# Aster32/GAN-DANet

Hardware: AMD Instinct MI355X
Metric: train samples/sec (G+D step) on 256x256 tiles (higher is better)
Workload: dtype bf16; 1 GPU; full G+D train step, 8ch 256x256 -> 1024x1024 tiles, batch 32/GPU (global 32), perceptual=on, SSIM evaluated, AdamW x2; survey_config=3, per_gpu_batch=32, global_batch=32, tile=256, parallelism=dp1

## Files before the change

### gan-danet_amd/_lib.py

```python
from __future__ import annotations

import ctypes as C
import os

HERE = os.path.dirname(os.path.abspath(__file__))
LIB_PATH = os.path.join(HERE, "lib", "libgandanet_hip.so")

PREC_FP32, PREC_BF16, PREC_X3 = 0, 1, 2
PAM_BWD_K64_ATOMIC, PAM_BWD_K64_PARTS, PAM_BWD_K32_PARTS, PAM_BWD_TWO_KERNEL = 0, 1, 2, 3
ACT_NONE, ACT_RELU, ACT_LEAKY02, ACT_SIGMOID = 0, 1, 2, 3
EVAL_F64, EVAL_SKIP_NAN = 1, 2
GUARD_SQNORM, GUARD_NORM, GUARD_COEF, GUARD_OK, GUARD_APPLIED, GUARD_SKIPPED, GUARD_RECORD = range(7)
GUARD_CHUNK = 65536
FILTER_F32, FILTER_F64 = 0, 1
EDGE_REFLECT, EDGE_INTERIOR = 0, 1
FILTER_MAX_RADIUS, SAVGOL_MAX_WINDOW = 64, 33
ZOOM_MIRROR, ZOOM_NEAREST = 0, 1

c_fp = C.c_void_p


class ConvDesc(C.Structure):
    _fields_ = [
        ("B", C.c_int), ("M", C.c_int), ("Mstore", C.c_int), ("Ck", C.c_int), ("ks", C.c_int),
# ... 41 lines not shown
    "gd_gemm_nt_plan": (_i, [C.POINTER(GemmNTDesc), _sz, C.POINTER(_i), C.POINTER(_sz)]),
    "gd_conv3x3_ws_bytes": (_sz, [_i, _i]),
    "gd_conv3x3_eligible": (_i, [C.POINTER(ConvDesc)]),
    "gd_conv3x3": (_i, [C.POINTER(ConvDesc), _p, _sz, _p]),
    "gd_conv3x3_wgrad": (_i, [_p, _l, _p, _p, _l, _p, _i, _p, _p, _i, _i, _i, _i, _i, _i, _i, _i, _p, _p]),
    "gd_conv3x3_wgrad_ws": (_i, [_p, _l, _p, _p, _l, _p, _i, _p, _p, _i, _i, _i, _i, _i, _i, _i, _i, _p, _p, _p, _sz]),
    "gd_conv3x3_wgrad_plan": (_i, [_i, _i, _i, _i, _i, _i, _sz, C.POINTER(_i), C.POINTER(_sz)]),
    "gd_pack_16_split": (_i, [_p, _l, _i, _i, _i, _p, _p, _i, _p, _l, _i, _l, _i, _i, _p, _l, _i, _l, _i, _i, _p]),
    "gd_pack_16_split_masked": (_i, [_p, _l, _i, _i, _i, _p, _p, _i, _p, _l, _i, _l, _i, _i, _p, _l, _i, _l, _i, _i, _p, _l, _p]),
    "gd_split3_weights": (_i, [_p, _l, _l, _l, _p, _p]),
    "gd_bn_stats_ws_floats": (_sz, [_i, _i, _l]),
    "gd_bn_stats": (_i, [_p, _l, _i, _i, _l, _f, _f, _p, _p, _p, _p, _p, _p]),
    "gd_bn_fold": (_i, [_p, _p, _p, _p, _i, _p, _p, _p]),
    "gd_bn_fold_eval": (_i, [_p, _p, _p, _p, _f, _i, _p, _p, _p, _p]),
    "gd_affine_act": (_i, [_p, _l, _p, _p, _i, _i, _l, _i, _p, _l, _p]),
    "gd_bn_act_bwd": (_i, [_p, _l, _p, _l, _p, _p, _p, _p, _p, _i, _i, _l, _i, _i, _p, _p, _p, _l, _i, _p, _p]),
    "gd_bn_stats_local": (_i, [_p, _l, _i, _i, _l, _p, _p, _p]),
    "gd_bn_stats_merge": (_i, [_p, _i, _i, _f, _f, _p, _p, _p, _p, _p]),
    "gd_bn_act_bwd_dx": (_i, [_p, _l, _p, _l, _p, _p, _p, _p, _p, _p, _f, _i, _i, _l, _i, _p, _l, _i, _p]),
    "gd_bicubic_fwd": (_i, [_p, _i, _i, _i, _p, _i, _i, _f, _f, _p]),
    "gd_bicubic_bwd": (_i, [_p, _i, _i, _i, _p, _i, _i, _f, _f, _p]),
    "gd_bilinear_fwd": (_i, [_p, _i, _i, _i, _p, _i, _i, _i, _p, _p]),
    "gd_bilinear_bwd": (_i, [_p, _i, _i, _i, _p, _i, _i, _p]),
    "gd_maxpool2_fwd": (_i, [_p, _i, _i, _i, _p, _p]),
    "gd_maxpool2_bwd": (_i, [_p, _p, _i, _i, _i, _p, _p]),
    "gd_act_fwd": (_i, [_p, _p, _l, _i, _p]),
    "gd_act_bwd": (_i, [_p, _p, _p, _l, _i, _p]),
    "gd_axpby": (_i, [_p, _f, _p, _f, _l, _p]),
    "gd_scale_dev": (_i, [_p, _p, _p, _l, _i, _p]),
    "gd_copy_rows": (_i, [_p, _l, _l, _p, _l, _l, _i, _i, _i, _p]),
    "gd_channel_sum": (_i, [_p, _l, _i, _i, _l, _p, _i, _p, _p]),
    "gd_copy_slab": (_i, [_p, _l, _p, _l, _i, _l, _i, _p]),
    "gd_softmax_rows": (_i, [_p, _p, _l, _i, _f, _p]),
    "gd_softmax_rows_bwd": (_i, [_p, _p, _p, _l, _i, _f, _p]),
# ... 131 lines not shown
```

### gan-danet_amd/csrc/norm.hip

```cpp
#include "common.h"
#include "../../include/gandanet.h"

namespace {

constexpr int CHUNK = 16384;

static inline int chunks_per_image(long HW) { return (int)((HW + CHUNK - 1) / CHUNK); }

__global__ __launch_bounds__(256) void bn_partial_kernel(const float* __restrict__ x, long x_bs, int C, long HW,
                                                        int cpi, float* __restrict__ ws) {
    __shared__ float red[8];
    const int c = blockIdx.x;
    const int part = blockIdx.y;
    const int b = part / cpi, j = part - b * cpi;
    const long i0 = (long)j * CHUNK;
    const long i1 = min(HW, i0 + (long)CHUNK);
    const float* p = x + (long)b * x_bs + (long)c * HW;
    const float shift = p[i0];
    float s1 = 0.f, s2 = 0.f;
    for (long i = i0 + threadIdx.x; i < i1; i += 256) {
        const float v = p[i] - shift;
        s1 += v;
        s2 = fmaf(v, v, s2);
    }
    s1 = gd_block_sum(s1, red);
    s2 = gd_block_sum(s2, red);
    if (threadIdx.x == 0) {
        const float n = (float)(i1 - i0);
        float* o = ws + ((long)c * gridDim.y + part) * 3;
        o[0] = n;
        o[1] = shift + s1 / n;
        o[2] = fmaxf(s2 - s1 * s1 / n, 0.f);
    }
}

__global__ __launch_bounds__(256) void bn_finalize_kernel(const float* __restrict__ ws, int parts, long c_stride,
                                                         long p_stride, float eps, float momentum,
                                                         float* __restrict__ mean, float* __restrict__ invstd,
                                                         float* running_mean, float* running_var,
                                                         float* __restrict__ stats_out) {
    __shared__ double redd[4];
    const int c = blockIdx.x;
    const float* w0 = ws + (long)c * c_stride * 3;
    const long ps = p_stride * 3;
    double n = 0, sm = 0;
    for (int i = threadIdx.x; i < parts; i += 256) {
        const float* w = w0 + i * ps;
        n += w[0];
        sm += (double)w[0] * w[1];
    }
    auto bsum = [&](double v) {
        v = gd_wave_sum_d(v);
        __syncthreads();
// ... 7 lines not shown
    double m2 = 0;
    for (int i = threadIdx.x; i < parts; i += 256) {
        const float* w = w0 + i * ps;
        const double dm = (double)w[1] - mu;
        m2 += (double)w[2] + (double)w[0] * dm * dm;
    }
    m2 = bsum(m2);
    if (threadIdx.x == 0 && stats_out) {
        stats_out[c * 3 + 0] = (float)n;
        stats_out[c * 3 + 1] = (float)mu;
        stats_out[c * 3 + 2] = (float)m2;
    } else if (threadIdx.x == 0) {
        const double var = m2 / n;
        mean[c] = (float)mu;
        invstd[c] = (float)(1.0 / sqrt(var + (double)eps));
        if (running_mean) {
            const double unb = n > 1 ? m2 / (n - 1) : var;
            running_mean[c] = (float)((1.0 - momentum) * running_mean[c] + momentum * mu);
            running_var[c] = (float)((1.0 - momentum) * running_var[c] + momentum * unb);
        }
    }
}

__global__ __launch_bounds__(256) void chan_sum_partial_kernel(const float* __restrict__ x, long x_bs, long HW, int cpi,
                                                              float* __restrict__ ws) {
    __shared__ float red[8];
    const int c = blockIdx.x;
    const int part = blockIdx.y;
    const int b = part / cpi, j = part - b * cpi;
    const long i0 = (long)j * CHUNK, i1 = min(HW, i0 + (long)CHUNK);
    const float* p = x + (long)b * x_bs + (long)c * HW;
    float s = 0.f;
    for (long i = i0 + threadIdx.x; i < i1; i += 256) s += p[i];
    s = gd_block_sum(s, red);
    if (threadIdx.x == 0) ws[(long)c * gridDim.y + part] = s;
// ... 113 lines not shown
    };
    a = bsum(a);
    g = bsum(g);
    if (threadIdx.x == 0) {
        dbeta[c] = (float)a;
        dgamma[c] = (float)g;
    }
}

__global__ __launch_bounds__(256) void bn_bwd_dx_kernel(const float* __restrict__ dy, long dy_bs,
                                                       const float* __restrict__ x, long x_bs,
                                                       const float* __restrict__ scale, const float* __restrict__ shift,
                                                       const float* __restrict__ mean, const float* __restrict__ invstd,
                                                       const float* __restrict__ dgamma, const float* __restrict__ dbeta,
                                                       float inv_n, long HW, int cpi, int act, int train,
                                                       float* __restrict__ dx, long dx_bs, int accumulate) {
    const int c = blockIdx.x;
    const int b = blockIdx.y / cpi, j = blockIdx.y - b * cpi;
    const long i0 = (long)j * CHUNK, i1 = min(HW, i0 + (long)CHUNK);
    const float* px = x + (long)b * x_bs + (long)c * HW;
    const float* pd = dy + (long)b * dy_bs + (long)c * HW;
    float* po = dx + (long)b * dx_bs + (long)c * HW;
    const float sc = scale[c], sh = shift[c], mu = mean[c], is = invstd[c];
    const float k_db = train ? dbeta[c] * inv_n : 0.f;
    const float k_dg = train ? dgamma[c] * inv_n : 0.f;
    for (long i = i0 + threadIdx.x; i < i1; i += 256) {
        const float xv = px[i];
        const float g = act_grad(fmaf(xv, sc, sh), pd[i], act);
        const float xh = (xv - mu) * is;
        float v = sc * (g - k_db - xh * k_dg);
        if (accumulate) v += po[i];
        po[i] = v;
    }
}

}

extern "C" size_t gd_bn_stats_ws_floats(int B, int C, long HW) {
    return (size_t)C * (size_t)B * (size_t)chunks_per_image(HW) * 3;
}

extern "C" int gd_bn_stats(const float* x, long x_bs, int B, int C, long HW, float eps, float momentum, float* mean,
                           float* invstd, float* running_mean, float* running_var, float* ws, void* stream) {
    GD_CHECK_ARG(x && mean && invstd && ws, "gd_bn_stats: null pointer");
    GD_CHECK_ARG(B > 0 && C > 0 && HW > 0, "gd_bn_stats: bad sizes");
    GD_CHECK_ARG((running_mean == nullptr) == (running_var == nullptr), "gd_bn_stats: running stats must come together");
    const int cpi = chunks_per_image(HW);
    GD_CHECK_ARG((long)B * cpi <= 65535, "gd_bn_stats: too many parts");
    hipStream_t s = (hipStream_t)stream;
    hipLaunchKernelGGL(bn_partial_kernel, dim3(C, B * cpi), dim3(256), 0, s, x, x_bs, C, HW, cpi, ws);
    hipLaunchKernelGGL(bn_finalize_kernel, dim3(C), dim3(256), 0, s, ws, B * cpi, (long)B * cpi, 1L, eps, momentum, mean, invstd,
                       running_mean, running_var, (float*)nullptr);
    GD_LAUNCH_CHECK();
    return 0;
}

extern "C" int gd_bn_stats_local(const float* x, long x_bs, int B, int C, long HW, float* stats, float* ws, void* stream) {
    GD_CHECK_ARG(x && stats && ws && B > 0 && C > 0 && HW > 0, "gd_bn_stats_local: bad arguments");
    const int cpi = chunks_per_image(HW);
    GD_CHECK_ARG((long)B * cpi <= 65535, "gd_bn_stats_local: too many parts");
    hipStream_t s = (hipStream_t)stream;
    hipLaunchKernelGGL(bn_partial_kernel, dim3(C, B * cpi), dim3(256), 0, s, x, x_bs, C, HW, cpi, ws);
    hipLaunchKernelGGL(bn_finalize_kernel, dim3(C), dim3(256), 0, s, ws, B * cpi, (long)B * cpi, 1L, 0.f, 0.f, (float*)nullptr,
                       (float*)nullptr, (float*)nullptr, (float*)nullptr, stats);
    GD_LAUNCH_CHECK();
    return 0;
}
extern "C" int gd_bn_stats_merge(const float* stats_all, int world, int C, float eps, float momentum, float* mean,
                                 float* invstd, float* running_mean, float* running_var, void* stream) {
    GD_CHECK_ARG(stats_all && mean && invstd && world > 0 && C > 0, "gd_bn_stats_merge: bad arguments");
    GD_CHECK_ARG((running_mean == nullptr) == (running_var == nullptr), "gd_bn_stats_merge: running stats must come together");
    hipLaunchKernelGGL(bn_finalize_kernel, dim3(C), dim3(256), 0, (hipStream_t)stream, stats_all, world, 1L, (long)C, eps,
                       momentum, mean, invstd, running_mean, running_var, (float*)nullptr);
    GD_LAUNCH_CHECK();
    return 0;
}

extern "C" int gd_channel_sum(const float* x, long x_bs, int B, int C, long HW, float* out, int accumulate, float* ws,
                              void* stream) {
    GD_CHECK_ARG(x && out && ws && B > 0 && C > 0 && HW > 0, "gd_channel_sum: bad arguments");
    const int cpi = chunks_per_image(HW);
    GD_CHECK_ARG((long)B * cpi <= 65535, "gd_channel_sum: too many parts");
    hipStream_t s = (hipStream_t)stream;
    hipLaunchKernelGGL(chan_sum_partial_kernel, dim3(C, B * cpi), dim3(256), 0, s, x, x_bs, HW, cpi, ws);
    hipLaunchKernelGGL(chan_sum_final_kernel, dim3(C), dim3(256), 0, s, ws, B * cpi, out, accumulate);
    GD_LAUNCH_CHECK();
    return 0;
}
// ... 19 lines not shown

extern "C" int gd_affine_act(const float* x, long x_bs, const float* scale, const float* shift, int B, int C, long HW,
                             int act, float* y, long y_bs, void* stream) {
    GD_CHECK_ARG(x && y && B > 0 && C > 0 && HW > 0, "gd_affine_act: bad arguments");
    const int cpi = chunks_per_image(HW);
    GD_CHECK_ARG((long)B * cpi <= 65535, "gd_affine_act: too many parts");
    hipLaunchKernelGGL(affine_act_kernel, dim3(C, B * cpi), dim3(256), 0, (hipStream_t)stream, x, x_bs, scale, shift, HW,
                       cpi, act, y, y_bs);
    GD_LAUNCH_CHECK();
    return 0;
}

extern "C" int gd_bn_act_bwd_dx(const float* dy, long dy_bs, const float* x, long x_bs, const float* scale, const float* shift,
                                const float* mean, const float* invstd, const float* dgamma_sum, const float* dbeta_sum,
                                float inv_n, int B, int C, long HW, int act, float* dx, long dx_bs, int accumulate_dx,
                                void* stream) {
    GD_CHECK_ARG(dy && x && scale && shift && mean && invstd && dgamma_sum && dbeta_sum && dx, "gd_bn_act_bwd_dx: null pointer");
    GD_CHECK_ARG(B > 0 && C > 0 && HW > 0 && inv_n > 0.f, "gd_bn_act_bwd_dx: bad sizes");
    const int cpi = chunks_per_image(HW);
    GD_CHECK_ARG((long)B * cpi <= 65535, "gd_bn_act_bwd_dx: too many parts");
    hipLaunchKernelGGL(bn_bwd_dx_kernel, dim3(C, B * cpi), dim3(256), 0, (hipStream_t)stream, dy, dy_bs, x, x_bs, scale, shift, mean,
                       invstd, dgamma_sum, dbeta_sum, inv_n, HW, cpi, act, 1, dx, dx_bs, accumulate_dx);
    GD_LAUNCH_CHECK();
    return 0;
}

extern "C" int gd_bn_act_bwd(const float* dy, long dy_bs, const float* x, long x_bs, const float* scale,
                             const float* shift, const float* mean, const float* invstd, const float* gamma, int B, int C,
                             long HW, int act, int train, float* dgamma, float* dbeta, float* dx, long dx_bs,
                             int accumulate_dx, float* ws, void* stream) {
    (void)gamma;
    GD_CHECK_ARG(dy && x && scale && shift && mean && invstd && dgamma && dbeta && ws, "gd_bn_act_bwd: null pointer");
    GD_CHECK_ARG(B > 0 && C > 0 && HW > 0, "gd_bn_act_bwd: bad sizes");
    const int cpi = chunks_per_image(HW);
    GD_CHECK_ARG((long)B * cpi <= 65535, "gd_bn_act_bwd: too many parts");
    hipStream_t s = (hipStream_t)stream;
    hipLaunchKernelGGL(bn_bwd_partial_kernel, dim3(C, B * cpi), dim3(256), 0, s, dy, dy_bs, x, x_bs, scale, shift, mean,
                       invstd, HW, cpi, act, ws);
    hipLaunchKernelGGL(bn_bwd_finalize_kernel, dim3(C), dim3(256), 0, s, ws, B * cpi, dgamma, dbeta);
    if (dx) {
        const float inv_n = 1.0f / ((float)B * (float)HW);
        hipLaunchKernelGGL(bn_bwd_dx_kernel, dim3(C, B * cpi), dim3(256), 0, s, dy, dy_bs, x, x_bs, scale, shift, mean,
                           invstd, dgamma, dbeta, inv_n, HW, cpi, act, train, dx, dx_bs, accumulate_dx);
    }
    GD_LAUNCH_CHECK();
    return 0;
}
```

### gan-danet_amd/kern.py

```python
from __future__ import annotations

import ctypes as C
import math
import os
from typing import Optional, Tuple

import torch

from . import _lib as L

Tensor = torch.Tensor


def _stream() -> int:
    return torch.cuda.current_stream().cuda_stream


def _ptr(t: Optional[Tensor]):
    return None if t is None else t.data_ptr()


def _chk(t: Tensor, name: str = "tensor", dtype=torch.float32) -> None:
    if not t.is_cuda:
        raise L.GandanetError(f"{name}: expected a GPU tensor (there is no CPU fallback in the product path)")
# ... 224 lines not shown
    return out


def bn_stats(x: Tensor, eps: float, momentum: float, running_mean: Optional[Tensor],
             running_var: Optional[Tensor]) -> Tuple[Tensor, Tensor]:
    bs = _bview(x, "bn input")
    B, Cn = x.shape[0], x.shape[1]
    HW = x[0, 0].numel()
    mean = torch.empty(Cn, device=x.device, dtype=torch.float32)
    invstd = torch.empty_like(mean)
    L.check(lib().gd_bn_stats(_ptr(x), bs, B, Cn, HW, eps, momentum, _ptr(mean), _ptr(invstd), _ptr(running_mean),
                              _ptr(running_var), _ptr(bn_ws(B, Cn, HW, x.device)), _stream()), "gd_bn_stats")
    return mean, invstd


def bn_stats_local(x: Tensor) -> Tensor:
    bs = _bview(x, "bn input")
    B, Cn = x.shape[0], x.shape[1]
    HW = x[0, 0].numel()
    stats = torch.empty(Cn, 3, device=x.device, dtype=torch.float32)
    L.check(lib().gd_bn_stats_local(_ptr(x), bs, B, Cn, HW, _ptr(stats), _ptr(bn_ws(B, Cn, HW, x.device)), _stream()),
            "gd_bn_stats_local")
    return stats


def bn_stats_merge(stats_all: Tensor, eps: float, momentum: float, running_mean: Optional[Tensor],
                   running_var: Optional[Tensor]) -> Tuple[Tensor, Tensor]:
    _dense(stats_all, "gathered BN records")
    world, Cn, _ = stats_all.shape
    mean = torch.empty(Cn, device=stats_all.device, dtype=torch.float32)
    invstd = torch.empty_like(mean)
    L.check(lib().gd_bn_stats_merge(_ptr(stats_all), world, Cn, eps, momentum, _ptr(mean), _ptr(invstd), _ptr(running_mean),
                                    _ptr(running_var), _stream()), "gd_bn_stats_merge")
    return mean, invstd


def bn_act_bwd_dx(dy: Tensor, x: Tensor, scale: Tensor, shift: Tensor, mean: Tensor, invstd: Tensor, dgamma_sum: Tensor,
                  dbeta_sum: Tensor, inv_n: float, act: int, dx: Optional[Tensor] = None, accumulate_dx: bool = False) -> Tensor:
    dbs, xbs = _bview(dy, "bn dy"), _bview(x, "bn x")
    B, Cn = x.shape[0], x.shape[1]
    HW = x[0, 0].numel()
    if dx is None:
        dx = torch.empty(x.shape, device=x.device, dtype=torch.float32)
        accumulate_dx = False
    L.check(lib().gd_bn_act_bwd_dx(_ptr(dy), dbs, _ptr(x), xbs, _ptr(scale), _ptr(shift), _ptr(mean), _ptr(invstd),
                                   _ptr(dgamma_sum), _ptr(dbeta_sum), float(inv_n), B, Cn, HW, act, _ptr(dx), _bview(dx),
                                   int(accumulate_dx), _stream()), "gd_bn_act_bwd_dx")
    return dx


def bn_fold(gamma: Tensor, beta: Tensor, mean: Tensor, invstd: Tensor) -> Tuple[Tensor, Tensor]:
    scale, shift = torch.empty_like(gamma), torch.empty_like(gamma)
    L.check(lib().gd_bn_fold(_ptr(gamma), _ptr(beta), _ptr(mean), _ptr(invstd), gamma.numel(), _ptr(scale),
                             _ptr(shift), _stream()), "gd_bn_fold")
    return scale, shift


def bn_fold_eval(gamma: Tensor, beta: Tensor, running_mean: Tensor, running_var: Tensor, eps: float):
    scale, shift, invstd = torch.empty_like(gamma), torch.empty_like(gamma), torch.empty_like(gamma)
    L.check(lib().gd_bn_fold_eval(_ptr(gamma), _ptr(beta), _ptr(running_mean), _ptr(running_var), eps,
                                  gamma.numel(), _ptr(scale), _ptr(shift), _ptr(invstd), _stream()), "gd_bn_fold_eval")
    return scale, shift, invstd


def affine_act(x: Tensor, scale: Optional[Tensor], shift: Optional[Tensor], act: int,
               out: Optional[Tensor] = None) -> Tensor:
    bs = _bview(x, "affine input")
    B, Cn = x.shape[0], x.shape[1]
    HW = x[0, 0].numel()
    if out is None:
        out = torch.empty(x.shape, device=x.device, dtype=torch.float32)
    L.check(lib().gd_affine_act(_ptr(x), bs, _ptr(scale), _ptr(shift), B, Cn, HW, act, _ptr(out), _bview(out),
                                _stream()), "gd_affine_act")
    return out


def bn_act_bwd(dy: Tensor, x: Tensor, scale: Tensor, shift: Tensor, mean: Tensor, invstd: Tensor, act: int,
               train: bool, dx: Optional[Tensor] = None, accumulate_dx: bool = False, want_dx: bool = True,
               sums_out: Optional[Tensor] = None):
    dbs, xbs = _bview(dy, "bn dy"), _bview(x, "bn x")
    B, Cn = x.shape[0], x.shape[1]
    HW = x[0, 0].numel()
    if sums_out is not None:
        dgamma, dbeta = _dense(sums_out)[0], sums_out[1]
    else:
        dgamma = torch.empty(Cn, device=x.device, dtype=torch.float32)
        dbeta = torch.empty_like(dgamma)
    if want_dx and dx is None:
        dx = torch.empty(x.shape, device=x.device, dtype=torch.float32)
    L.check(lib().gd_bn_act_bwd(_ptr(dy), dbs, _ptr(x), xbs, _ptr(scale), _ptr(shift), _ptr(mean), _ptr(invstd), None,
                                B, Cn, HW, act, int(train), _ptr(dgamma), _ptr(dbeta), _ptr(dx) if want_dx else None,
                                _bview(dx) if want_dx else 0, int(accumulate_dx), _ptr(bn_ws(B, Cn, HW, x.device)),
                                _stream()), "gd_bn_act_bwd")
    return dgamma, dbeta, dx


def bicubic_fwd(x: Tensor, Ho: int, Wo: int, rsh: float, rsw: float) -> Tensor:
    _dense(x, "bicubic input")
    B, Cn, Hi, Wi = x.shape
    y = torch.empty(B, Cn, Ho, Wo, device=x.device, dtype=torch.float32)
    L.check(lib().gd_bicubic_fwd(_ptr(x), B * Cn, Hi, Wi, _ptr(y), Ho, Wo, rsh, rsw, _stream()), "gd_bicubic_fwd")
    return y


def shift_sum9_fwd(u: Tensor, bias: Optional[Tensor]) -> Tensor:
    _dense(u, "tap planes")
    B, nine, H, W = u.shape
    if nine != 9:
# ... 1120 lines not shown
```

### gan-danet_amd/ops.py

```python
from __future__ import annotations

import os
from typing import List, Optional

import torch
from torch.autograd import Function

from . import _lib as L
from . import kern as K
from .config import config, operand_mode, sixteen_bit

ACT_NONE, ACT_RELU, ACT_LEAKY, ACT_SIGMOID = L.ACT_NONE, L.ACT_RELU, L.ACT_LEAKY02, L.ACT_SIGMOID


def _prec(layer: str = "other") -> int:
    mode = operand_mode(layer)
    return L.PREC_BF16 if mode == "16" else L.PREC_X3 if mode == "x3" else L.PREC_FP32


def _x3(layer: str) -> bool:
    return operand_mode(layer) == "x3"


def _x3_eligible(x, w, stride, pad, act) -> bool:
    return (x.dim() == 4 and tuple(w.shape[2:]) == (3, 3) and stride == 1 and pad == 1 and act in (ACT_NONE, ACT_RELU)
            and w.shape[1] >= 32 and w.shape[1] % 8 == 0 and w.shape[0] % 8 == 0 and (x.shape[2] * x.shape[3]) % 8 == 0
            and x.shape[2] * x.shape[3] * 3 * max(w.shape[0], w.shape[1]) < (1 << 31))


def _pam_f16() -> bool:
    return config.precision in ("fp16", "mixed")


def _c(t: torch.Tensor) -> torch.Tensor:
    return t if t.is_contiguous() else t.contiguous()


DISC_NHWC = os.environ.get("GD_DISC_NHWC", "1") != "0"


def disc1_trunk_eligible(x: torch.Tensor, ws) -> bool:
    return (DISC_NHWC and (sixteen_bit("disc") or _x3("disc")) and (not K.DETERMINISTIC or K.DET_REDUCE == "ordered")
            and x.dim() == 4 and x.shape[1] <= 4
            and ws[0].shape[0] == 64 and all(w.shape[0] % 8 == 0 and w.shape[2:] == (3, 3) for w in ws))


class Disc1TrunkFn(Function):

    SLOPE = 0.2

# ... 162 lines not shown


def _bn_prepare(x, gamma, beta, rmean, rvar, training, momentum, eps):
    if training and _sync_bn_active():
        mean, invstd = K.bn_stats_merge(_all_gather_records(K.bn_stats_local(x)), eps, momentum, rmean, rvar)
        scale, shift = K.bn_fold(gamma, beta, mean, invstd)
    elif training:
        mean, invstd = K.bn_stats(x, eps, momentum, rmean, rvar)
        scale, shift = K.bn_fold(gamma, beta, mean, invstd)
    else:
        scale, shift, invstd = K.bn_fold_eval(gamma, beta, rmean, rvar, eps)
        mean = rmean
    return scale, shift, mean, invstd


def _bn_bwd(dy, x, scale, shift, mean, invstd, act, training, sync, dx=None, accumulate_dx=False):
    if not (sync and training):
        return K.bn_act_bwd(dy, x, scale, shift, mean, invstd, act, training, dx=dx, accumulate_dx=accumulate_dx)
    import torch.distributed as dist
    Cn = x.shape[1]
    sums = torch.empty(2, Cn, device=x.device, dtype=torch.float32)
    K.bn_act_bwd(dy, x, scale, shift, mean, invstd, act, training, want_dx=False, sums_out=sums)
    local = torch.empty_like(sums)
    K.copy_slab(sums.view(1, 2 * Cn, 1), local.view(1, 2 * Cn, 1))
    dist.all_reduce(sums, op=dist.ReduceOp.SUM)
    n_global = x.shape[0] * x[0, 0].numel() * dist.get_world_size()
    dx = K.bn_act_bwd_dx(dy, x, scale, shift, mean, invstd, sums[0], sums[1], 1.0 / n_global, act, dx=dx,
                         accumulate_dx=accumulate_dx)
    return local[0], local[1], dx


class BnActFn(Function):
    @staticmethod
    def forward(ctx, x, gamma, beta, rmean, rvar, training: bool, momentum: float, eps: float, act: int):
        scale, shift, mean, invstd = _bn_prepare(x, gamma, beta, rmean, rvar, training, momentum, eps)
        y = K.affine_act(x, scale, shift, act)
        ctx.save_for_backward(x, scale, shift, mean, invstd)
        ctx.cfg = (act, training, training and _sync_bn_active())
        return y

    @staticmethod
    def backward(ctx, dy):
        x, scale, shift, mean, invstd = ctx.saved_tensors
        act, training, sync = ctx.cfg
        dgamma, dbeta, dx = _bn_bwd(_c(dy), x, scale, shift, mean, invstd, act, training, sync)
        return dx, dgamma, dbeta, None, None, None, None, None, None


def batch_norm_act(x, gamma, beta, rmean, rvar, training, momentum, eps, act=ACT_NONE):
    return BnActFn.apply(x, gamma, beta, rmean, rvar, training, momentum, eps, act)


class BnReluConvFn(Function):

    @staticmethod
    def forward(ctx, x, gamma, beta, rmean, rvar, w, bias, training, momentum, eps, pad):
        prec = _prec("conv1x1" if w.shape[2] == 1 else "other")
        scale, shift, mean, invstd = _bn_prepare(x, gamma, beta, rmean, rvar, training, momentum, eps)
        y = K.conv2d_fwd(x, w, bias, 1, pad, prec, in_scale=scale, in_shift=shift, in_relu=True)
        ctx.save_for_backward(x, scale, shift, mean, invstd, w)
        ctx.cfg = (training, prec, pad, bias is not None, training and _sync_bn_active())
        return y

    @staticmethod
    def backward(ctx, dy):
        x, scale, shift, mean, invstd, w = ctx.saved_tensors
        training, prec, pad, has_bias, sync = ctx.cfg
        dy = _c(dy)
        dw = K.conv2d_wgrad(dy, x, w.shape[2], 1, pad, prec, in_scale=scale, in_shift=shift, in_relu=True)
        db = K.channel_sum(dy) if has_bias else None
        dxt = K.conv2d_dgrad(dy, w, (x.shape[2], x.shape[3]), 1, pad, prec)
        dgamma, dbeta, dx = _bn_bwd(dxt, x, scale, shift, mean, invstd, ACT_RELU, training, sync)
        return dx, dgamma, dbeta, None, None, dw, db, None, None, None, None


class DenseBlockFn(Function):

    @staticmethod
    def forward(ctx, x, training: bool, momentum: float, eps: float, *params):
        prec = _prec("dense3x3")
        nl = len(params) // 6
        B, C0, H, W = x.shape
        g = params[4].shape[0]
        slab = torch.empty(B, C0 + nl * g, H, W, device=x.device, dtype=torch.float32)
        K.copy_slab(x, slab[:, :C0])
        saved: List[torch.Tensor] = []
        aligned = ((H * W) % 8 == 0 and g % 8 == 0 and all((C0 + l * g) % 8 == 0 for l in range(nl))
                   and tuple(params[4].shape[2:]) == (3, 3))
        split = prec == L.PREC_X3 and aligned and C0 >= 32 and H * W * 3 * (C0 + nl * g) < (1 << 31)
        packed = split or (DENSE_NHWC and prec == L.PREC_BF16 and aligned)
        packs: List[torch.Tensor] = []
        for l in range(nl):
            bw, bb, rm, rv, cw, cb = params[6 * l: 6 * l + 6]
            cl = C0 + l * g
            xin = slab[:, :cl]
            scale, shift, mean, invstd = _bn_prepare(xin, bw, bb, rm, rv, training, momentum, eps)
            if packed:
                packs.append(_pack3x3_x(xin, split, scale, shift, relu=True))
                _packed3x3_fwd(packs[-1], cw, cb, H, W, split, out=slab[:, cl:cl + g])
            else:
                K.conv2d_fwd(xin, cw, cb, 1, 1, prec, in_scale=scale, in_shift=shift, in_relu=True,
                             out=slab[:, cl:cl + g])
            saved += [scale, shift, mean, invstd, cw]
        ctx.save_for_backward(slab, *saved, *packs)
        ctx.cfg = (nl, C0, g, training, prec, [p is not None for p in params[5::6]], packed, split, training and _sync_bn_active())
        return slab

    @staticmethod
    def backward(ctx, dslab_in):
        slab, *saved = ctx.saved_tensors
        nl, C0, g, training, prec, has_bias, packed, split, sync = ctx.cfg
        packs = saved[5 * nl:]
        B, _, H, W = slab.shape
        dslab = torch.empty(slab.shape, device=slab.device, dtype=torch.float32)
        K.copy_slab(_c(dslab_in), dslab)
        grads: List[Optional[torch.Tensor]] = [None] * (6 * nl)
        for l in reversed(range(nl)):
            scale, shift, mean, invstd, cw = saved[5 * l: 5 * l + 5]
            cl = C0 + l * g
            xin = slab[:, :cl]
            dy = dslab[:, cl:cl + g]
            if packed:
                dxt, grads[6 * l + 4] = _packed3x3_bwd(dy, packs[l], cw, H, W, split, True, True, dw_first=True)
            else:
                grads[6 * l + 4] = K.conv2d_wgrad(dy, xin, 3, 1, 1, prec, in_scale=scale, in_shift=shift, in_relu=True)
                dxt = K.conv2d_dgrad(dy, cw, (H, W), 1, 1, prec)
            if has_bias[l]:
                grads[6 * l + 5] = K.channel_sum(dy)
            dgamma, dbeta, _ = _bn_bwd(dxt, xin, scale, shift, mean, invstd, ACT_RELU, training, sync,
                                       dx=dslab[:, :cl], accumulate_dx=True)
            grads[6 * l + 0], grads[6 * l + 1] = dgamma, dbeta
        dx = torch.empty(B, C0, H, W, device=slab.device, dtype=torch.float32)
        K.copy_slab(dslab[:, :C0], dx)
        return (dx, None, None, None, *grads)


def _npad(n: int) -> int:
    return (n + 255) // 256 * 256


def _cp(c: int) -> int:
    return (c + 31) // 32 * 32


def _pam_wide(Cn: int, r: int) -> bool:
    return K.PAM_WIDE and sixteen_bit("pam") and 192 < Cn <= 511 and r <= 63


def _pam_f32(B: int, Cn: int, r: int, N: int) -> bool:
# ... 780 lines not shown
```

### include/gandanet.h

```cpp
#ifndef GANDANET_H
#define GANDANET_H
#include <stddef.h>
#include <stdint.h>
#ifdef __cplusplus
extern "C" {
#endif

#define GD_VERSION 100
void gd_set_deterministic(int on);
int gd_get_deterministic(void);
int gd_set_det_reduce(int mode);
int gd_get_det_reduce(void);
int gd_version(void);
int gd_last_error(char* buf, int n);
int gd_sizeof_conv_desc(void);
int gd_sizeof_gemm_nt_desc(void);

enum { GD_PREC_FP32 = 0,
       GD_PREC_BF16 = 1,
       GD_PREC_X3 = 2     };
enum { GD_ACT_NONE = 0, GD_ACT_RELU = 1, GD_ACT_LEAKY02 = 2, GD_ACT_SIGMOID = 3 };

typedef struct gd_conv_desc {
    int B;
// ... 39 lines not shown
    const float* in_scale; const float* in_shift; int in_relu;
    float* c; long c_bs, ldc;
    const float* alpha;
    const float* bias;
    int accumulate;
    int splits;
    int precision;
} gd_gemm_nt_desc;
int gd_gemm_nt(const gd_gemm_nt_desc* d, void* stream);
int gd_gemm_nt_ws(const gd_gemm_nt_desc* d, void* stream, void* ws, size_t ws_bytes);
int gd_gemm_nt_plan(const gd_gemm_nt_desc* d, size_t ws_bytes, int* splits, size_t* ws_needed);

size_t gd_bn_stats_ws_floats(int B, int C, long HW);
int gd_bn_stats(const float* x, long x_bs, int B, int C, long HW, float eps, float momentum,
                float* mean, float* invstd, float* running_mean, float* running_var, float* ws, void* stream);
int gd_bn_fold(const float* gamma, const float* beta, const float* mean, const float* invstd, int C,
               float* scale, float* shift, void* stream);
int gd_bn_stats_local(const float* x, long x_bs, int B, int C, long HW, float* stats, float* ws, void* stream);
int gd_bn_stats_merge(const float* stats_all, int world, int C, float eps, float momentum, float* mean, float* invstd,
                      float* running_mean, float* running_var, void* stream);
int gd_bn_act_bwd_dx(const float* dy, long dy_bs, const float* x, long x_bs, const float* scale, const float* shift,
                     const float* mean, const float* invstd, const float* dgamma_sum, const float* dbeta_sum, float inv_n,
                     int B, int C, long HW, int act, float* dx, long dx_bs, int accumulate_dx, void* stream);
int gd_bn_fold_eval(const float* gamma, const float* beta, const float* running_mean, const float* running_var,
                    float eps, int C, float* scale, float* shift, float* invstd_out, void* stream);
int gd_channel_sum(const float* x, long x_bs, int B, int C, long HW, float* out, int accumulate, float* ws,
                   void* stream);
int gd_affine_act(const float* x, long x_bs, const float* scale, const float* shift, int B, int C, long HW,
                  int act, float* y, long y_bs, void* stream);
int gd_bn_act_bwd(const float* dy, long dy_bs, const float* x, long x_bs, const float* scale, const float* shift,
                  const float* mean, const float* invstd, const float* gamma, int B, int C, long HW, int act,
                  int train, float* dgamma, float* dbeta, float* dx, long dx_bs, int accumulate_dx, float* ws,
                  void* stream);

int gd_bicubic_fwd(const float* x, int BC, int Hi, int Wi, float* y, int Ho, int Wo, float rscale_h,
                   float rscale_w, void* stream);
int gd_bicubic_bwd(const float* dy, int BC, int Hi, int Wi, float* dx, int Ho, int Wo, float rscale_h,
                   float rscale_w, void* stream);
int gd_shift_sum9_fwd(const float* u, const float* bias, float* y, int B, int H, int W, void* stream);
int gd_shift_sum9_bwd(const float* dy, float* du, int B, int H, int W, void* stream);
int gd_combine_inputs(const float* lr, int C1, int H1, int W1, float rs1, const float* aux, int C2, int H2, int W2,
                      float rs2, float* out, int B, int Ho, int Wo, void* stream);
int gd_bilinear_fwd(const float* x, int BC, int Hi, int Wi, float* y, int Ho, int Wo, int accumulate,
                    const float* res, void* stream);
int gd_bilinear_bwd(const float* dy, int BC, int Hi, int Wi, float* dx, int Ho, int Wo, void* stream);
int gd_maxpool2_fwd(const float* x, int BC, int Hi, int Wi, float* y, void* stream);
int gd_maxpool2_bwd(const float* x, const float* dy, int BC, int Hi, int Wi, float* dx, void* stream);

// ... 186 lines not shown
```

Before: 36.60 samples/s.

## Reuse per-channel BN moments across dense block layers and fuse residual grad copy

In the dense block forward, per-channel batch-norm moments are now computed once per new channel slab and cached, instead of re-reducing the whole growing concatenated input at every layer. Running statistics are updated by a new small kernel from the cached mean/var/count. In backward, the initial copy of the incoming gradient into a full slab and the final copy-out are removed: the last layer reads the incoming gradient directly and the BN backward kernel gains a residual input so dx = bn_grad + res is written in one pass. This changes the reduction order of statistics slightly and adds API surface.

```diff
diff --git a/gan-danet_amd/_lib.py b/gan-danet_amd/_lib.py
--- a/gan-danet_amd/_lib.py
+++ b/gan-danet_amd/_lib.py
@@ -79,10 +79,13 @@
     "gd_bn_fold": (_i, [_p, _p, _p, _p, _i, _p, _p, _p]),
     "gd_bn_fold_eval": (_i, [_p, _p, _p, _p, _f, _i, _p, _p, _p, _p]),
     "gd_affine_act": (_i, [_p, _l, _p, _p, _i, _i, _l, _i, _p, _l, _p]),
-    "gd_bn_act_bwd": (_i, [_p, _l, _p, _l, _p, _p, _p, _p, _p, _i, _i, _l, _i, _i, _p, _p, _p, _l, _i, _p, _p]),
+    "gd_bn_stats_moments": (_i, [_p, _l, _i, _i, _l, _i, _i, _f, _p, _p, _p, _p, _p, _p]),
+    "gd_bn_running_update": (_i, [_p, _p, _p, _f, _p, _p, _i, _p]),
+    "gd_bn_stats_merge_moments": (_i, [_p, _i, _i, _f, _p, _p, _p, _p, _p]),
+    "gd_bn_act_bwd": (_i, [_p, _l, _p, _l, _p, _p, _p, _p, _p, _i, _i, _l, _i, _i, _p, _p, _p, _l, _i, _p, _l, _p, _p]),
     "gd_bn_stats_local": (_i, [_p, _l, _i, _i, _l, _p, _p, _p]),
     "gd_bn_stats_merge": (_i, [_p, _i, _i, _f, _f, _p, _p, _p, _p, _p]),
-    "gd_bn_act_bwd_dx": (_i, [_p, _l, _p, _l, _p, _p, _p, _p, _p, _p, _f, _i, _i, _l, _i, _p, _l, _i, _p]),
+    "gd_bn_act_bwd_dx": (_i, [_p, _l, _p, _l, _p, _p, _p, _p, _p, _p, _f, _i, _i, _l, _i, _p, _l, _i, _p, _l, _p]),
     "gd_bicubic_fwd": (_i, [_p, _i, _i, _i, _p, _i, _i, _f, _f, _p]),
     "gd_bicubic_bwd": (_i, [_p, _i, _i, _i, _p, _i, _i, _f, _f, _p]),
     "gd_bilinear_fwd": (_i, [_p, _i, _i, _i, _p, _i, _i, _i, _p, _p]),
diff --git a/gan-danet_amd/csrc/norm.hip b/gan-danet_amd/csrc/norm.hip
--- a/gan-danet_amd/csrc/norm.hip
+++ b/gan-danet_amd/csrc/norm.hip
@@ -34,9 +34,25 @@
     }
 }
 
+__device__ __forceinline__ void bn_running_blend(float mean, float var, float count, float momentum, float* running_mean,
+                                                 float* running_var) {
+    const double n = (double)count, m = (double)momentum;
+    const double unb = n > 1 ? (double)var * (n / (n - 1)) : (double)var;
+    *running_mean = (float)fma(m, (double)mean, (1.0 - m) * (double)*running_mean);
+    *running_var = (float)fma(m, unb, (1.0 - m) * (double)*running_var);
+}
+
+__global__ void bn_running_update_kernel(const float* __restrict__ mean, const float* __restrict__ var,
+                                         const float* __restrict__ count, float momentum, float* running_mean,
+                                         float* running_var, int C) {
+    const int c = blockIdx.x * blockDim.x + threadIdx.x;
+    if (c < C) bn_running_blend(mean[c], var[c], count[c], momentum, running_mean + c, running_var + c);
+}
+
 __global__ __launch_bounds__(256) void bn_finalize_kernel(const float* __restrict__ ws, int parts, long c_stride,
                                                          long p_stride, float eps, float momentum,
                                                          float* __restrict__ mean, float* __restrict__ invstd,
+                                                         float* __restrict__ var_out, float* __restrict__ count_out,
                                                          float* running_mean, float* running_var,
                                                          float* __restrict__ stats_out) {
     __shared__ double redd[4];
@@ -74,11 +90,9 @@
         const double var = m2 / n;
         mean[c] = (float)mu;
         invstd[c] = (float)(1.0 / sqrt(var + (double)eps));
-        if (running_mean) {
-            const double unb = n > 1 ? m2 / (n - 1) : var;
-            running_mean[c] = (float)((1.0 - momentum) * running_mean[c] + momentum * mu);
-            running_var[c] = (float)((1.0 - momentum) * running_var[c] + momentum * unb);
-        }
+        if (var_out) var_out[c] = (float)var;
+        if (count_out) count_out[c] = (float)n;
+        if (running_mean) bn_running_blend((float)mu, (float)var, (float)n, momentum, running_mean + c, running_var + c);
     }
 }
 
@@ -222,13 +236,15 @@
                                                        const float* __restrict__ mean, const float* __restrict__ invstd,
                                                        const float* __restrict__ dgamma, const float* __restrict__ dbeta,
                                                        float inv_n, long HW, int cpi, int act, int train,
-                                                       float* __restrict__ dx, long dx_bs, int accumulate) {
+                                                       float* __restrict__ dx, long dx_bs, int accumulate,
+                                                       const float* __restrict__ res, long res_bs) {
     const int c = blockIdx.x;
     const int b = blockIdx.y / cpi, j = blockIdx.y - b * cpi;
     const long i0 = (long)j * CHUNK, i1 = min(HW, i0 + (long)CHUNK);
     const float* px = x + (long)b * x_bs + (long)c * HW;
     const float* pd = dy + (long)b * dy_bs + (long)c * HW;
     float* po = dx + (long)b * dx_bs + (long)c * HW;
+    const float* pa = res ? res + (long)b * res_bs + (long)c * HW : accumulate ? po : nullptr;
     const float sc = scale[c], sh = shift[c], mu = mean[c], is = invstd[c];
     const float k_db = train ? dbeta[c] * inv_n : 0.f;
     const float k_dg = train ? dgamma[c] * inv_n : 0.f;
@@ -237,7 +253,7 @@
         const float g = act_grad(fmaf(xv, sc, sh), pd[i], act);
         const float xh = (xv - mu) * is;
         float v = sc * (g - k_db - xh * k_dg);
-        if (accumulate) v += po[i];
+        if (pa) v += pa[i];
         po[i] = v;
     }
 }
@@ -246,6 +262,15 @@
 
 extern "C" size_t gd_bn_stats_ws_floats(int B, int C, long HW) {
     return (size_t)C * (size_t)B * (size_t)chunks_per_image(HW) * 3;
+}
+
+static void launch_bn_reduce(const float* x, long x_bs, int B, int C, long HW, float eps, float momentum, float* mean,
+                             float* invstd, float* var, float* count, float* running_mean, float* running_var,
+                             float* stats, float* ws, hipStream_t s) {
+    const int cpi = chunks_per_image(HW);
+    hipLaunchKernelGGL(bn_partial_kernel, dim3(C, B * cpi), dim3(256), 0, s, x, x_bs, C, HW, cpi, ws);
+    hipLaunchKernelGGL(bn_finalize_kernel, dim3(C), dim3(256), 0, s, ws, B * cpi, (long)B * cpi, 1L, eps, momentum, mean, invstd,
+                       var, count, running_mean, running_var, stats);
 }
 
 extern "C" int gd_bn_stats(const float* x, long x_bs, int B, int C, long HW, float eps, float momentum, float* mean,
@@ -253,33 +278,63 @@
     GD_CHECK_ARG(x && mean && invstd && ws, "gd_bn_stats: null pointer");
     GD_CHECK_ARG(B > 0 && C > 0 && HW > 0, "gd_bn_stats: bad sizes");
     GD_CHECK_ARG((running_mean == nullptr) == (running_var == nullptr), "gd_bn_stats: running stats must come together");
-    const int cpi = chunks_per_image(HW);
-    GD_CHECK_ARG((long)B * cpi <= 65535, "gd_bn_stats: too many parts");
-    hipStream_t s = (hipStream_t)stream;
-    hipLaunchKernelGGL(bn_partial_kernel, dim3(C, B * cpi), dim3(256), 0, s, x, x_bs, C, HW, cpi, ws);
-    hipLaunchKernelGGL(bn_finalize_kernel, dim3(C), dim3(256), 0, s, ws, B * cpi, (long)B * cpi, 1L, eps, momentum, mean, invstd,
-                       running_mean, running_var, (float*)nullptr);
+    GD_CHECK_ARG((long)B * chunks_per_image(HW) <= 65535, "gd_bn_stats: too many parts");
+    launch_bn_reduce(x, x_bs, B, C, HW, eps, momentum, mean, invstd, nullptr, nullptr, running_mean, running_var, nullptr, ws,
+                     (hipStream_t)stream);
+    GD_LAUNCH_CHECK();
+    return 0;
+}
+
+extern "C" int gd_bn_stats_moments(const float* x, long x_bs, int B, int C_total, long HW, int c0, int C, float eps,
+                                   float* mean, float* var, float* invstd, float* count, float* ws, void* stream) {
+    GD_CHECK_ARG(x && mean && var && invstd && count && ws, "gd_bn_stats_moments: null pointer");
+    GD_CHECK_ARG(B > 0 && C > 0 && C_total > 0 && HW > 0, "gd_bn_stats_moments: bad sizes (C <= 0?)");
+    GD_CHECK_ARG(c0 >= 0 && (long)c0 + C <= C_total, "gd_bn_stats_moments: channel range outside the tensor");
+    GD_CHECK_ARG(B == 1 || x_bs >= (long)C_total * HW, "gd_bn_stats_moments: batch stride below one image");
+    GD_CHECK_ARG((long)B * chunks_per_image(HW) <= 65535, "gd_bn_stats_moments: too many parts");
+    launch_bn_reduce(x + (long)c0 * HW, x_bs, B, C, HW, eps, 0.f, mean, invstd, var, count, nullptr, nullptr, nullptr, ws,
+                     (hipStream_t)stream);
+    GD_LAUNCH_CHECK();
+    return 0;
+}
+
+extern "C" int gd_bn_running_update(const float* mean, const float* var, const float* count, float momentum,
+                                    float* running_mean, float* running_var, int C, void* stream) {
+    GD_CHECK_ARG(mean && var && count && running_mean && running_var, "gd_bn_running_update: null pointer");
+    GD_CHECK_ARG(C > 0, "gd_bn_running_update: C <= 0");
+    hipLaunchKernelGGL(bn_running_update_kernel, dim3(gd_cdiv(C, 256)), dim3(256), 0, (hipStream_t)stream, mean, var, count,
+                       momentum, running_mean, running_var, C);
     GD_LAUNCH_CHECK();
     return 0;
 }
 
 extern "C" int gd_bn_stats_local(const float* x, long x_bs, int B, int C, long HW, float* stats, float* ws, void* stream) {
     GD_CHECK_ARG(x && stats && ws && B > 0 && C > 0 && HW > 0, "gd_bn_stats_local: bad arguments");
-    const int cpi = chunks_per_image(HW);
-    GD_CHECK_ARG((long)B * cpi <= 65535, "gd_bn_stats_local: too many parts");
-    hipStream_t s = (hipStream_t)stream;
-    hipLaunchKernelGGL(bn_partial_kernel, dim3(C, B * cpi), dim3(256), 0, s, x, x_bs, C, HW, cpi, ws);
-    hipLaunchKernelGGL(bn_finalize_kernel, dim3(C), dim3(256), 0, s, ws, B * cpi, (long)B * cpi, 1L, 0.f, 0.f, (float*)nullptr,
-                       (float*)nullptr, (float*)nullptr, (float*)nullptr, stats);
-    GD_LAUNCH_CHECK();
-    return 0;
+    GD_CHECK_ARG((long)B * chunks_per_image(HW) <= 65535, "gd_bn_stats_local: too many parts");
+    launch_bn_reduce(x, x_bs, B, C, HW, 0.f, 0.f, nullptr, nullptr, nullptr, nullptr, nullptr, nullptr, stats, ws,
+                     (hipStream_t)stream);
+    GD_LAUNCH_CHECK();
+    return 0;
+}
+static void launch_bn_merge(const float* stats_all, int world, int C, float eps, float momentum, float* mean, float* invstd,
+                            float* var, float* count, float* running_mean, float* running_var, hipStream_t s) {
+    hipLaunchKernelGGL(bn_finalize_kernel, dim3(C), dim3(256), 0, s, stats_all, world, 1L, (long)C, eps, momentum, mean, invstd,
+                       var, count, running_mean, running_var, (float*)nullptr);
 }
 extern "C" int gd_bn_stats_merge(const float* stats_all, int world, int C, float eps, float momentum, float* mean,
                                  float* invstd, float* running_mean, float* running_var, void* stream) {
     GD_CHECK_ARG(stats_all && mean && invstd && world > 0 && C > 0, "gd_bn_stats_merge: bad arguments");
     GD_CHECK_ARG((running_mean == nullptr) == (running_var == nullptr), "gd_bn_stats_merge: running stats must come together");
-    hipLaunchKernelGGL(bn_finalize_kernel, dim3(C), dim3(256), 0, (hipStream_t)stream, stats_all, world, 1L, (long)C, eps,
-                       momentum, mean, invstd, running_mean, running_var, (float*)nullptr);
+    launch_bn_merge(stats_all, world, C, eps, momentum, mean, invstd, nullptr, nullptr, running_mean, running_var,
+                    (hipStream_t)stream);
+    GD_LAUNCH_CHECK();
+    return 0;
+}
+extern "C" int gd_bn_stats_merge_moments(const float* stats_all, int world, int C, float eps, float* mean, float* var,
+                                         float* invstd, float* count, void* stream) {
+    GD_CHECK_ARG(stats_all && mean && var && invstd && count, "gd_bn_stats_merge_moments: null pointer");
+    GD_CHECK_ARG(world > 0 && C > 0, "gd_bn_stats_merge_moments: bad sizes (C <= 0?)");
+    launch_bn_merge(stats_all, world, C, eps, 0.f, mean, invstd, var, count, nullptr, nullptr, (hipStream_t)stream);
     GD_LAUNCH_CHECK();
     return 0;
 }
@@ -329,13 +384,15 @@
 extern "C" int gd_bn_act_bwd_dx(const float* dy, long dy_bs, const float* x, long x_bs, const float* scale, const float* shift,
                                 const float* mean, const float* invstd, const float* dgamma_sum, const float* dbeta_sum,
                                 float inv_n, int B, int C, long HW, int act, float* dx, long dx_bs, int accumulate_dx,
-                                void* stream) {
+                                const float* res, long res_bs, void* stream) {
     GD_CHECK_ARG(dy && x && scale && shift && mean && invstd && dgamma_sum && dbeta_sum && dx, "gd_bn_act_bwd_dx: null pointer");
     GD_CHECK_ARG(B > 0 && C > 0 && HW > 0 && inv_n > 0.f, "gd_bn_act_bwd_dx: bad sizes");
+    GD_CHECK_ARG(!(res && accumulate_dx), "gd_bn_act_bwd_dx: res and accumulate_dx exclude each other");
+    GD_CHECK_ARG(!res || (res != dx && (B == 1 || res_bs >= (long)C * HW)), "gd_bn_act_bwd_dx: bad res");
     const int cpi = chunks_per_image(HW);
     GD_CHECK_ARG((long)B * cpi <= 65535, "gd_bn_act_bwd_dx: too many parts");
     hipLaunchKernelGGL(bn_bwd_dx_kernel, dim3(C, B * cpi), dim3(256), 0, (hipStream_t)stream, dy, dy_bs, x, x_bs, scale, shift, mean,
-                       invstd, dgamma_sum, dbeta_sum, inv_n, HW, cpi, act, 1, dx, dx_bs, accumulate_dx);
+                       invstd, dgamma_sum, dbeta_sum, inv_n, HW, cpi, act, 1, dx, dx_bs, accumulate_dx, res, res_bs);
     GD_LAUNCH_CHECK();
     return 0;
 }
@@ -343,10 +400,12 @@
 extern "C" int gd_bn_act_bwd(const float* dy, long dy_bs, const float* x, long x_bs, const float* scale,
                              const float* shift, const float* mean, const float* invstd, const float* gamma, int B, int C,
                              long HW, int act, int train, float* dgamma, float* dbeta, float* dx, long dx_bs,
-                             int accumulate_dx, float* ws, void* stream) {
+                             int accumulate_dx, const float* res, long res_bs, float* ws, void* stream) {
     (void)gamma;
     GD_CHECK_ARG(dy && x && scale && shift && mean && invstd && dgamma && dbeta && ws, "gd_bn_act_bwd: null pointer");
     GD_CHECK_ARG(B > 0 && C > 0 && HW > 0, "gd_bn_act_bwd: bad sizes");
+    GD_CHECK_ARG(!res || (dx && !accumulate_dx), "gd_bn_act_bwd: res needs dx and excludes accumulate_dx");
+    GD_CHECK_ARG(!res || (res != dx && (B == 1 || res_bs >= (long)C * HW)), "gd_bn_act_bwd: bad res");
     const int cpi = chunks_per_image(HW);
     GD_CHECK_ARG((long)B * cpi <= 65535, "gd_bn_act_bwd: too many parts");
     hipStream_t s = (hipStream_t)stream;
@@ -356,8 +415,8 @@
     if (dx) {
         const float inv_n = 1.0f / ((float)B * (float)HW);
         hipLaunchKernelGGL(bn_bwd_dx_kernel, dim3(C, B * cpi), dim3(256), 0, s, dy, dy_bs, x, x_bs, scale, shift, mean,
-                           invstd, dgamma, dbeta, inv_n, HW, cpi, act, train, dx, dx_bs, accumulate_dx);
-    }
-    GD_LAUNCH_CHECK();
-    return 0;
-}
+                           invstd, dgamma, dbeta, inv_n, HW, cpi, act, train, dx, dx_bs, accumulate_dx, res, res_bs);
+    }
+    GD_LAUNCH_CHECK();
+    return 0;
+}
diff --git a/gan-danet_amd/kern.py b/gan-danet_amd/kern.py
--- a/gan-danet_amd/kern.py
+++ b/gan-danet_amd/kern.py
@@ -262,6 +262,46 @@
     return mean, invstd
 
 
+def bn_stats_moments(x: Tensor, c0: int, c1: int, eps: float, out=None):
+    bs = _bview(x, "bn input")
+    B, Ct = x.shape[0], x.shape[1]
+    HW = x[0, 0].numel()
+    Cn = c1 - c0
+    if out is None:
+        out = tuple(torch.empty(max(Cn, 0), device=x.device, dtype=torch.float32) for _ in range(4))
+    mean, var, invstd, count = out
+    for t in out:
+        if _dense(t, "bn moments").numel() != Cn:
+            raise L.GandanetError("bn_stats_moments: output vectors must hold one value per channel of the range")
+    L.check(lib().gd_bn_stats_moments(_ptr(x), bs, B, Ct, HW, c0, Cn, eps, _ptr(mean), _ptr(var), _ptr(invstd), _ptr(count),
+                                      _ptr(bn_ws(B, max(Cn, 1), HW, x.device)), _stream()), "gd_bn_stats_moments")
+    return mean, var, invstd, count
+
+
+def bn_running_update(mean: Tensor, var: Tensor, count: Tensor, momentum: float, running_mean: Tensor,
+                      running_var: Tensor) -> None:
+    Cn = running_mean.numel()
+    for t in (mean, var, count, running_mean, running_var):
+        if _dense(t, "bn moments").numel() != Cn:
+            raise L.GandanetError("bn_running_update: vectors of different lengths")
+    L.check(lib().gd_bn_running_update(_ptr(mean), _ptr(var), _ptr(count), momentum, _ptr(running_mean), _ptr(running_var),
+                                       Cn, _stream()), "gd_bn_running_update")
+
+
+def bn_stats_merge_moments(stats_all: Tensor, eps: float, out=None):
+    _dense(stats_all, "gathered BN records")
+    world, Cn, _ = stats_all.shape
+    if out is None:
+        out = tuple(torch.empty(Cn, device=stats_all.device, dtype=torch.float32) for _ in range(4))
+    mean, var, invstd, count = out
+    for t in out:
+        if _dense(t, "bn moments").numel() != Cn:
+            raise L.GandanetError("bn_stats_merge_moments: output vectors must hold one value per channel")
+    L.check(lib().gd_bn_stats_merge_moments(_ptr(stats_all), world, Cn, eps, _ptr(mean), _ptr(var), _ptr(invstd), _ptr(count),
+                                            _stream()), "gd_bn_stats_merge_moments")
+    return mean, var, invstd, count
+
+
 def bn_stats_local(x: Tensor) -> Tensor:
     bs = _bview(x, "bn input")
     B, Cn = x.shape[0], x.shape[1]
@@ -284,7 +324,8 @@
 
 
 def bn_act_bwd_dx(dy: Tensor, x: Tensor, scale: Tensor, shift: Tensor, mean: Tensor, invstd: Tensor, dgamma_sum: Tensor,
-                  dbeta_sum: Tensor, inv_n: float, act: int, dx: Optional[Tensor] = None, accumulate_dx: bool = False) -> Tensor:
+                  dbeta_sum: Tensor, inv_n: float, act: int, dx: Optional[Tensor] = None, accumulate_dx: bool = False,
+                  res: Optional[Tensor] = None) -> Tensor:
     dbs, xbs = _bview(dy, "bn dy"), _bview(x, "bn x")
     B, Cn = x.shape[0], x.shape[1]
     HW = x[0, 0].numel()
@@ -293,8 +334,16 @@
         accumulate_dx = False
     L.check(lib().gd_bn_act_bwd_dx(_ptr(dy), dbs, _ptr(x), xbs, _ptr(scale), _ptr(shift), _ptr(mean), _ptr(invstd),
                                    _ptr(dgamma_sum), _ptr(dbeta_sum), float(inv_n), B, Cn, HW, act, _ptr(dx), _bview(dx),
-                                   int(accumulate_dx), _stream()), "gd_bn_act_bwd_dx")
+                                   int(accumulate_dx), _ptr(res), _res_bs(res, x), _stream()), "gd_bn_act_bwd_dx")
     return dx
+
+
+def _res_bs(res: Optional[Tensor], x: Tensor) -> int:
+    if res is None:
+        return 0
+    if res.shape != x.shape:
+        raise L.GandanetError("bn backward: res must have the shape of x")
+    return _bview(res, "bn res")
 
 
 def bn_fold(gamma: Tensor, beta: Tensor, mean: Tensor, invstd: Tensor) -> Tuple[Tensor, Tensor]:
@@ -325,7 +374,7 @@
 
 def bn_act_bwd(dy: Tensor, x: Tensor, scale: Tensor, shift: Tensor, mean: Tensor, invstd: Tensor, act: int,
                train: bool, dx: Optional[Tensor] = None, accumulate_dx: bool = False, want_dx: bool = True,
-               sums_out: Optional[Tensor] = None):
+               sums_out: Optional[Tensor] = None, res: Optional[Tensor] = None):
     dbs, xbs = _bview(dy, "bn dy"), _bview(x, "bn x")
     B, Cn = x.shape[0], x.shape[1]
     HW = x[0, 0].numel()
@@ -338,8 +387,8 @@
         dx = torch.empty(x.shape, device=x.device, dtype=torch.float32)
     L.check(lib().gd_bn_act_bwd(_ptr(dy), dbs, _ptr(x), xbs, _ptr(scale), _ptr(shift), _ptr(mean), _ptr(invstd), None,
                                 B, Cn, HW, act, int(train), _ptr(dgamma), _ptr(dbeta), _ptr(dx) if want_dx else None,
-                                _bview(dx) if want_dx else 0, int(accumulate_dx), _ptr(bn_ws(B, Cn, HW, x.device)),
-                                _stream()), "gd_bn_act_bwd")
+                                _bview(dx) if want_dx else 0, int(accumulate_dx), _ptr(res), _res_bs(res, x),
+                                _ptr(bn_ws(B, Cn, HW, x.device)), _stream()), "gd_bn_act_bwd")
     return dgamma, dbeta, dx
 
 
diff --git a/gan-danet_amd/ops.py b/gan-danet_amd/ops.py
--- a/gan-danet_amd/ops.py
+++ b/gan-danet_amd/ops.py
@@ -34,6 +34,14 @@
 
 def _c(t: torch.Tensor) -> torch.Tensor:
     return t if t.is_contiguous() else t.contiguous()
+
+
+def _cb(t: torch.Tensor) -> torch.Tensor:
+    if t.dim() != 4 or t.is_contiguous():
+        return _c(t)
+    b, c, h, w = t.shape
+    ok = t.stride(3) == 1 and t.stride(2) == w and t.stride(1) == h * w and (b == 1 or t.stride(0) >= c * h * w)
+    return t if ok else t.contiguous()
 
 
 DISC_NHWC = os.environ.get("GD_DISC_NHWC", "1") != "0"
@@ -226,9 +234,9 @@
     return scale, shift, mean, invstd
 
 
-def _bn_bwd(dy, x, scale, shift, mean, invstd, act, training, sync, dx=None, accumulate_dx=False):
+def _bn_bwd(dy, x, scale, shift, mean, invstd, act, training, sync, dx=None, accumulate_dx=False, res=None):
     if not (sync and training):
-        return K.bn_act_bwd(dy, x, scale, shift, mean, invstd, act, training, dx=dx, accumulate_dx=accumulate_dx)
+        return K.bn_act_bwd(dy, x, scale, shift, mean, invstd, act, training, dx=dx, accumulate_dx=accumulate_dx, res=res)
     import torch.distributed as dist
     Cn = x.shape[1]
     sums = torch.empty(2, Cn, device=x.device, dtype=torch.float32)
@@ -238,7 +246,7 @@
     dist.all_reduce(sums, op=dist.ReduceOp.SUM)
     n_global = x.shape[0] * x[0, 0].numel() * dist.get_world_size()
     dx = K.bn_act_bwd_dx(dy, x, scale, shift, mean, invstd, sums[0], sums[1], 1.0 / n_global, act, dx=dx,
-                         accumulate_dx=accumulate_dx)
+                         accumulate_dx=accumulate_dx, res=res)
     return local[0], local[1], dx
 
 
@@ -255,7 +263,7 @@
     def backward(ctx, dy):
         x, scale, shift, mean, invstd = ctx.saved_tensors
         act, training, sync = ctx.cfg
-        dgamma, dbeta, dx = _bn_bwd(_c(dy), x, scale, shift, mean, invstd, act, training, sync)
+        dgamma, dbeta, dx = _bn_bwd(_cb(dy), x, scale, shift, mean, invstd, act, training, sync)
         return dx, dgamma, dbeta, None, None, None, None, None, None
 
 
@@ -278,7 +286,7 @@
     def backward(ctx, dy):
         x, scale, shift, mean, invstd, w = ctx.saved_tensors
         training, prec, pad, has_bias, sync = ctx.cfg
-        dy = _c(dy)
+        dy = _cb(dy)
         dw = K.conv2d_wgrad(dy, x, w.shape[2], 1, pad, prec, in_scale=scale, in_shift=shift, in_relu=True)
         db = K.channel_sum(dy) if has_bias else None
         dxt = K.conv2d_dgrad(dy, w, (x.shape[2], x.shape[3]), 1, pad, prec)
@@ -287,6 +295,14 @@
 
 
 class DenseBlockFn(Function):
+
+    @staticmethod
+    def _moments(slab, c0, c1, eps, sync, mom):
+        out = tuple(v[c0:c1] for v in mom)
+        if sync:
+            K.bn_stats_merge_moments(_all_gather_records(K.bn_stats_local(slab[:, c0:c1])), eps, out=out)
+        else:
+            K.bn_stats_moments(slab, c0, c1, eps, out=out)
 
     @staticmethod
     def forward(ctx, x, training: bool, momentum: float, eps: float, *params):
@@ -302,20 +318,32 @@
         split = prec == L.PREC_X3 and aligned and C0 >= 32 and H * W * 3 * (C0 + nl * g) < (1 << 31)
         packed = split or (DENSE_NHWC and prec == L.PREC_BF16 and aligned)
         packs: List[torch.Tensor] = []
+        sync = training and _sync_bn_active()
+        if training:
+            mom = tuple(torch.empty(C0 + (nl - 1) * g, device=x.device, dtype=torch.float32) for _ in range(4))
+            DenseBlockFn._moments(slab, 0, C0, eps, sync, mom)
         for l in range(nl):
             bw, bb, rm, rv, cw, cb = params[6 * l: 6 * l + 6]
             cl = C0 + l * g
             xin = slab[:, :cl]
-            scale, shift, mean, invstd = _bn_prepare(xin, bw, bb, rm, rv, training, momentum, eps)
+            if training:
+                mean, var, invstd, count = (v[:cl] for v in mom)
+                if rm is not None:
+                    K.bn_running_update(mean, var, count, momentum, rm, rv)
+                scale, shift = K.bn_fold(bw, bb, mean, invstd)
+            else:
+                scale, shift, mean, invstd = _bn_prepare(xin, bw, bb, rm, rv, False, momentum, eps)
             if packed:
                 packs.append(_pack3x3_x(xin, split, scale, shift, relu=True))
                 _packed3x3_fwd(packs[-1], cw, cb, H, W, split, out=slab[:, cl:cl + g])
             else:
                 K.conv2d_fwd(xin, cw, cb, 1, 1, prec, in_scale=scale, in_shift=shift, in_relu=True,
                              out=slab[:, cl:cl + g])
+            if training and l + 1 < nl:
+                DenseBlockFn._moments(slab, cl, cl + g, eps, sync, mom)
             saved += [scale, shift, mean, invstd, cw]
         ctx.save_for_backward(slab, *saved, *packs)
-        ctx.cfg = (nl, C0, g, training, prec, [p is not None for p in params[5::6]], packed, split, training and _sync_bn_active())
+        ctx.cfg = (nl, C0, g, training, prec, [p is not None for p in params[5::6]], packed, split, sync)
         return slab
 
     @staticmethod
@@ -324,14 +352,15 @@
         nl, C0, g, training, prec, has_bias, packed, split, sync = ctx.cfg
         packs = saved[5 * nl:]
         B, _, H, W = slab.shape
-        dslab = torch.empty(slab.shape, device=slab.device, dtype=torch.float32)
-        K.copy_slab(_c(dslab_in), dslab)
+        dslab_in = _cb(dslab_in)
+        dslab = torch.empty(B, C0 + (nl - 1) * g, H, W, device=slab.device, dtype=torch.float32)
         grads: List[Optional[torch.Tensor]] = [None] * (6 * nl)
         for l in reversed(range(nl)):
             scale, shift, mean, invstd, cw = saved[5 * l: 5 * l + 5]
             cl = C0 + l * g
             xin = slab[:, :cl]
-            dy = dslab[:, cl:cl + g]
+            last = l == nl - 1
+            dy = (dslab_in if last else dslab)[:, cl:cl + g]
             if packed:
                 dxt, grads[6 * l + 4] = _packed3x3_bwd(dy, packs[l], cw, H, W, split, True, True, dw_first=True)
             else:
@@ -339,12 +368,10 @@
                 dxt = K.conv2d_dgrad(dy, cw, (H, W), 1, 1, prec)
             if has_bias[l]:
                 grads[6 * l + 5] = K.channel_sum(dy)
-            dgamma, dbeta, _ = _bn_bwd(dxt, xin, scale, shift, mean, invstd, ACT_RELU, training, sync,
-                                       dx=dslab[:, :cl], accumulate_dx=True)
+            dgamma, dbeta, _ = _bn_bwd(dxt, xin, scale, shift, mean, invstd, ACT_RELU, training, sync, dx=dslab[:, :cl],
+                                       accumulate_dx=not last, res=dslab_in[:, :cl] if last else None)
             grads[6 * l + 0], grads[6 * l + 1] = dgamma, dbeta
-        dx = torch.empty(B, C0, H, W, device=slab.device, dtype=torch.float32)
-        K.copy_slab(dslab[:, :C0], dx)
-        return (dx, None, None, None, *grads)
+        return (dslab[:, :C0], None, None, None, *grads)
 
 
 def _npad(n: int) -> int:
diff --git a/include/gandanet.h b/include/gandanet.h
--- a/include/gandanet.h
+++ b/include/gandanet.h
@@ -77,14 +77,21 @@
 size_t gd_bn_stats_ws_floats(int B, int C, long HW);
 int gd_bn_stats(const float* x, long x_bs, int B, int C, long HW, float eps, float momentum,
                 float* mean, float* invstd, float* running_mean, float* running_var, float* ws, void* stream);
+int gd_bn_stats_moments(const float* x, long x_bs, int B, int C_total, long HW, int c0, int C, float eps, float* mean,
+                        float* var, float* invstd, float* count, float* ws, void* stream);
+int gd_bn_running_update(const float* mean, const float* var, const float* count, float momentum, float* running_mean,
+                         float* running_var, int C, void* stream);
 int gd_bn_fold(const float* gamma, const float* beta, const float* mean, const float* invstd, int C,
                float* scale, float* shift, void* stream);
 int gd_bn_stats_local(const float* x, long x_bs, int B, int C, long HW, float* stats, float* ws, void* stream);
 int gd_bn_stats_merge(const float* stats_all, int world, int C, float eps, float momentum, float* mean, float* invstd,
                       float* running_mean, float* running_var, void* stream);
+int gd_bn_stats_merge_moments(const float* stats_all, int world, int C, float eps, float* mean, float* var, float* invstd,
+                              float* count, void* stream);
 int gd_bn_act_bwd_dx(const float* dy, long dy_bs, const float* x, long x_bs, const float* scale, const float* shift,
                      const float* mean, const float* invstd, const float* dgamma_sum, const float* dbeta_sum, float inv_n,
-                     int B, int C, long HW, int act, float* dx, long dx_bs, int accumulate_dx, void* stream);
+                     int B, int C, long HW, int act, float* dx, long dx_bs, int accumulate_dx, const float* res,
+                     long res_bs, void* stream);
 int gd_bn_fold_eval(const float* gamma, const float* beta, const float* running_mean, const float* running_var,
                     float eps, int C, float* scale, float* shift, float* invstd_out, void* stream);
 int gd_channel_sum(const float* x, long x_bs, int B, int C, long HW, float* out, int accumulate, float* ws,
@@ -93,8 +100,8 @@
                   int act, float* y, long y_bs, void* stream);
 int gd_bn_act_bwd(const float* dy, long dy_bs, const float* x, long x_bs, const float* scale, const float* shift,
                   const float* mean, const float* invstd, const float* gamma, int B, int C, long HW, int act,
-                  int train, float* dgamma, float* dbeta, float* dx, long dx_bs, int accumulate_dx, float* ws,
-                  void* stream);
+                  int train, float* dgamma, float* dbeta, float* dx, long dx_bs, int accumulate_dx, const float* res,
+                  long res_bs, float* ws, void* stream);
 
 int gd_bicubic_fwd(const float* x, int BC, int Hi, int Wi, float* y, int Ho, int Wo, float rscale_h,
                    float rscale_w, void* stream);
```

Result: no change. 36.73 samples/s (median of 6 runs) (+0.3%).
